# CITlabRostock/citlab-article-separation-new

Measured on AMD Instinct MI355X. Metric: newspaper pages/sec (ARU-Net seg + GNN relation) at 3000x4500 px, higher is better.
Workload: dtype f32s

## Files before the change

### citlab-article-separation-new_amd/csrc/aru_engine.hip

```cpp
#include <algorithm>
#include <cmath>
#include <cstdlib>
#include <memory>

#include "aru_kernels.h"
#include "res8_kernels.h"
#include "res8v_kernels.h"
#include "bf16_kernels.h"
#include "res8w_kernels.h"
#include "convr_kernels.h"
#include "split_kernels.h"
#include "asep_common.h"

using namespace asep;

namespace {

struct Tensor {
    float* p = nullptr;
    int H = 0, W = 0, C = 0;
    bool bf = false;
    size_t count() const { return (size_t)H * W * C; }
    bf16_t* bp() const { return reinterpret_cast<bf16_t*>(p); }
};

struct PackedConv {
    int kh = 0, kw = 0, cin = 0, cout = 0;
    bool c8 = false;
    bool c12 = false;
    bool deconv = false;
    int groups = 0, mtiles = 0, nchunks = 0;
    float* d_w = nullptr;
    float* d_b = nullptr;
    float* d_wino = nullptr;
    float* d_wv = nullptr;
    int bmode = -1;
    int bchunks = 0;
    bf16_t* d_wb = nullptr;
    bf16_t* d_wb8 = nullptr;
    int smode = -1;
    bf16_t* d_ws = nullptr;
    bf16_t* d_ws16 = nullptr;
// ... 15 lines not shown

struct asep_aru {
    asep_aru_cfg cfg{};
    std::map<std::string, PackedConv> convs;
    struct ResB { int C = 0; bf16_t* d_w = nullptr; float* d_b = nullptr; };
    std::map<std::string, ResB> resb;
    bf16_t* d_r8b_down_w = nullptr;
    float* d_r8b_down_b = nullptr;
    bf16_t* d_r8b_up_w1 = nullptr;
    bf16_t* d_r8f_up_w1 = nullptr;
    bf16_t* d_r8f_down_w1 = nullptr;
    float* d_r8b_down_w1r = nullptr;
    bool use_res32 = true;
    int walk_mode = 1;
    bool use_deconvs = true;
    bool use_convr = true;
    unsigned char* d_zero_trash = nullptr;
    int fused_act = 0;
    bool use_walk = true;
    bf16_t* d_r8b_up_w = nullptr;
    float* d_r8b_up_b = nullptr;
    float* d_r8b_up_b1 = nullptr;
    DirectConv det_first, att_first;
    float* d_r8_down_wr = nullptr;
    float* d_r8_down_br = nullptr;
    float* d_r8_up_w1 = nullptr;
    float* d_r8_up_wr = nullptr;
    float* d_r8_up_br = nullptr;
    float* d_r8_up_b1 = nullptr;
    float* d_r8v_down_wr = nullptr;
    float* d_r8v_up_w1 = nullptr;
    float* d_r8v_up_wr = nullptr;
    bool r8_valu = true;
    bool use_fused8 = true;
    bool fused8_wanted = true;
    bool fused8_var = false;
    float* d_att_head = nullptr;
    bf16_t* d_att_headb = nullptr;
    float* d_logit_w = nullptr;
    float* d_logit_b = nullptr;
    float* d_logit_wd = nullptr;
    float* d_stats = nullptr;
    double* d_sums = nullptr;
    struct Lane {
        hipStream_t s = nullptr;
        bool own_stream = false;
        hipStream_t side = nullptr;
        hipEvent_t ev_fork = nullptr, ev_join = nullptr, ev_begin = nullptr, ev_done = nullptr;
        hipStream_t bside = nullptr;
        hipEvent_t ev_bfork = nullptr, ev_bjoin = nullptr;
        BufferPool pool;
        ~Lane() {
            if (ev_fork) (void)hipEventDestroy(ev_fork);
            if (ev_bfork) (void)hipEventDestroy(ev_bfork);
            if (ev_bjoin) (void)hipEventDestroy(ev_bjoin);
            if (ev_join) (void)hipEventDestroy(ev_join);
            if (ev_begin) (void)hipEventDestroy(ev_begin);
            if (ev_done) (void)hipEventDestroy(ev_done);
            if (side) (void)hipStreamDestroy(side);
            if (bside) (void)hipStreamDestroy(bside);
            if (own_stream && s) (void)hipStreamDestroy(s);
        }
    };
    std::vector<std::unique_ptr<Lane>> lanes;
    Lane* cur = nullptr;
    int last_nl = 0;
// ... 732 lines not shown
        if (!rc) rc = upload(pwr, &m->d_r8_up_wr);
        if (!rc) rc = upload(pbr, &m->d_r8_up_br);
        if (!rc) rc = upload(b1->second.data, &m->d_r8_up_b1);
        if (!rc) rc = upload(vw1, &m->d_r8v_up_w1);
        if (!rc) rc = upload(vwr2, &m->d_r8v_up_wr);
        if (rc) return rc;
        m->owned.push_back(m->d_r8v_up_w1); m->owned.push_back(m->d_r8v_up_wr);
        m->owned.push_back(m->d_r8_up_w1); m->owned.push_back(m->d_r8_up_wr);
        m->owned.push_back(m->d_r8_up_br); m->owned.push_back(m->d_r8_up_b1);
        if (hipFuncSetAttribute((const void*)res8_up_kernel<false>, hipFuncAttributeMaxDynamicSharedMemorySize, (int)R8_UP_LDS) != hipSuccess ||
            hipFuncSetAttribute((const void*)res8v_up_kernel<0>, hipFuncAttributeMaxDynamicSharedMemorySize, (int)R8_UP_LDS) != hipSuccess ||
            hipFuncSetAttribute((const void*)res8v_up_kernel<1>, hipFuncAttributeMaxDynamicSharedMemorySize, (int)R8_UP_LDS) != hipSuccess ||
            hipFuncSetAttribute((const void*)res8v_up_kernel<2>, hipFuncAttributeMaxDynamicSharedMemorySize, (int)R8_UP_LDS) != hipSuccess) {
            set_error("cannot reserve %zu bytes of LDS for the fused up block", R8_UP_LDS);
            return ASEP_ERR_HIP;
        }
    }
    if (hipFuncSetAttribute((const void*)res8_down_kernel<false>, hipFuncAttributeMaxDynamicSharedMemorySize, (int)R8_DOWN_LDS) != hipSuccess ||
        hipFuncSetAttribute((const void*)res8v_down_kernel<0>, hipFuncAttributeMaxDynamicSharedMemorySize, (int)R8_DOWN_LDS) != hipSuccess ||
        hipFuncSetAttribute((const void*)res8v_down_kernel<1>, hipFuncAttributeMaxDynamicSharedMemorySize, (int)R8_DOWN_LDS) != hipSuccess ||
        hipFuncSetAttribute((const void*)res8v_down_kernel<2>, hipFuncAttributeMaxDynamicSharedMemorySize, (int)R8_DOWN_LDS) != hipSuccess) {
        set_error("cannot reserve %zu bytes of LDS for the fused residual block", R8_DOWN_LDS);
        return ASEP_ERR_HIP;
    }
    return ASEP_OK;
}

bool r8v_fits(const TL& l) {
    for (const Tensor& t : l)
        if ((size_t)t.H * t.W >= ((size_t)1 << 28)) return false;
    return true;
}

void run_res8_down(asep_aru* m, const TL& imgs, const std::vector<const float*>& stats, bool want_pool, TL* d_out, TL* pool_out) {
    for (const Tensor& t : imgs) {
        d_out->push_back(new_tensor(m, t.H, t.W, 8));
        if (want_pool) pool_out->push_back(new_tensor(m, cdiv(t.H, 2), cdiv(t.W, 2), 8));
    }
    for (size_t b0 = 0; b0 < imgs.size(); b0 += MAXP) {
        const size_t b1 = std::min(imgs.size(), b0 + MAXP);
        Res8Args a{};
        int tiles = 0;
        double flops = 0, bytes = 0;
        for (size_t i = b0; i < b1; ++i) {
            bytes += tbytes(imgs[i]) + tbytes((*d_out)[i]) + (want_pool ? tbytes((*pool_out)[i]) : 0.0);
            Res8Prob& p = a.p[i - b0];
            p.img = imgs[i].p; p.in1 = nullptr; p.stats = stats.empty() ? nullptr : stats[i];
            p.out = (*d_out)[i].p; p.pool = want_pool ? (*pool_out)[i].p : nullptr;
            p.H = imgs[i].H; p.W = imgs[i].W;
            p.tiles_x = cdiv(imgs[i].W, R8_OW);
            p.tile_begin = tiles;
            tiles += p.tiles_x * cdiv(imgs[i].H, R8_OH * R8_NP);
            flops += 2.0 * imgs[i].H * imgs[i].W * (9.0 * 8 + 3 * 9.0 * 64);
        }
        a.nprob = (int)(b1 - b0);
        a.total_tiles = tiles;
        a.w1 = m->det_first.d_w; a.b1 = m->det_first.d_b;
        bool valu = m->r8_valu;
        for (size_t i = b0; i < b1; ++i) valu = valu && (size_t)imgs[i].H * imgs[i].W < ((size_t)1 << 28);
        a.wr = (const f32x4*)(valu ? m->d_r8v_down_wr : m->d_r8_down_wr); a.br = m->d_r8_down_br;
        TL sub(imgs.begin() + b0, imgs.begin() + b1);
        const std::string pname = valu ? std::string("res8v_down_kernel<0>") : std::string("res8_down_kernel<false>");
        ProfScope ps(m, pname, flops, "unet_down_0 (conv1+3xconvR+add+pool) " + dims_of(sub));
        ps.bytes = bytes;
        a.sched = tile_schedule(m, a, std::min(tiles, m->num_cus), R8_OH * R8_NP);
        const dim3 gd(std::min(tiles, m->num_cus));
        const int actv = m->cfg.activation;
        if (actv && !valu) { set_error("level-0 block of an elu / leaky graph: image too large for the vector-ALU kernel"); throw ArgError(); }
        if (valu && actv == 1) { ps.set_name("res8v_down_kernel<1>"); hipLaunchKernelGGL(res8v_down_kernel<1>, gd, dim3(R8_THREADS), R8_DOWN_LDS, m->stream, a); }
        else if (valu && actv == 2) { ps.set_name("res8v_down_kernel<2>"); hipLaunchKernelGGL(res8v_down_kernel<2>, gd, dim3(R8_THREADS), R8_DOWN_LDS, m->stream, a); }
        else if (valu) hipLaunchKernelGGL(res8v_down_kernel<0>, gd, dim3(R8_THREADS), R8_DOWN_LDS, m->stream, a);
        else hipLaunchKernelGGL(res8_down_kernel<false>, gd, dim3(R8_THREADS), R8_DOWN_LDS, m->stream, a);
    }
}

TL run_res8_up(asep_aru* m, const TL& skip, const TL& v) {
    TL out;
    for (const Tensor& t : skip) out.push_back(new_tensor(m, t.H, t.W, 8));
    for (size_t b0 = 0; b0 < skip.size(); b0 += MAXP) {
        const size_t b1 = std::min(skip.size(), b0 + MAXP);
        Res8Args a{};
        int tiles = 0;
        double flops = 0, bytes = 0;
        for (size_t i = b0; i < b1; ++i) {
            bytes += tbytes(skip[i]) + tbytes(v[i]) + tbytes(out[i]);
            Res8Prob& p = a.p[i - b0];
            p.img = skip[i].p; p.in1 = v[i].p; p.stats = nullptr; p.out = out[i].p; p.pool = nullptr;
            p.H = skip[i].H; p.W = skip[i].W;
            p.tiles_x = cdiv(skip[i].W, R8_OW);
            p.tile_begin = tiles;
            tiles += p.tiles_x * cdiv(skip[i].H, R8_OH * R8_NP);
            flops += 2.0 * skip[i].H * skip[i].W * (9.0 * 16 * 8 + 3 * 9.0 * 64);
        }
        a.nprob = (int)(b1 - b0);
        a.total_tiles = tiles;
        bool valu = m->r8_valu;
        for (size_t i = b0; i < b1; ++i) valu = valu && (size_t)skip[i].H * skip[i].W < ((size_t)1 << 28);
        a.w1 = valu ? m->d_r8v_up_w1 : m->d_r8_up_w1; a.b1 = m->d_r8_up_b1;
        a.wr = (const f32x4*)(valu ? m->d_r8v_up_wr : m->d_r8_up_wr); a.br = m->d_r8_up_br;
        TL sub(skip.begin() + b0, skip.begin() + b1);
        const std::string pname = valu ? std::string("res8v_up_kernel<0>") : std::string("res8_up_kernel<false>");
        ProfScope ps(m, pname, flops, "unet_up_0 (conv1[16->8]+3xconvR+add) " + dims_of(sub));
        ps.bytes = bytes;
        a.sched = tile_schedule(m, a, std::min(tiles, m->num_cus), R8_OH * R8_NP);
        const dim3 grid(std::min(tiles, m->num_cus));
        const int actv = m->cfg.activation;
        if (actv && !valu) { set_error("level-0 block of an elu / leaky graph: image too large for the vector-ALU kernel"); throw ArgError(); }
        if (valu && actv == 1) { ps.set_name("res8v_up_kernel<1>"); hipLaunchKernelGGL(res8v_up_kernel<1>, grid, dim3(R8_THREADS), R8_UP_LDS, m->stream, a); }
        else if (valu && actv == 2) { ps.set_name("res8v_up_kernel<2>"); hipLaunchKernelGGL(res8v_up_kernel<2>, grid, dim3(R8_THREADS), R8_UP_LDS, m->stream, a); }
        else if (valu) hipLaunchKernelGGL(res8v_up_kernel<0>, grid, dim3(R8_THREADS), R8_UP_LDS, m->stream, a);
        else hipLaunchKernelGGL(res8_up_kernel<false>, grid, dim3(R8_THREADS), R8_UP_LDS, m->stream, a);
    }
    return out;
}

bf16_t f2bf(float f) {
    uint32_t u;
    memcpy(&u, &f, 4);
    u += 0x7fffu + ((u >> 16) & 1u);
    return (bf16_t)(u >> 16);
}

int upload_bf(const std::vector<bf16_t>& h, bf16_t** d) {
    ASEP_HIP_CHECK(hipMalloc((void**)d, std::max<size_t>(h.size(), 8) * sizeof(bf16_t)));
    ASEP_HIP_CHECK(hipMemcpy(*d, h.data(), h.size() * sizeof(bf16_t), hipMemcpyHostToDevice));
    return ASEP_OK;
}

template <class WF>
void pack_frags_conv(int mode, int kh, int kw, int cin, int mtiles, WF W, std::vector<bf16_t>& dst, int* nchunks) {
    const int taps = kh * kw;
    const int chunks = mode == 0 ? kh : (mode == 1 ? (taps + 1) / 2 : (cin / 32) * taps);
    *nchunks = chunks;
    for (int ch = 0; ch < chunks; ++ch)
        for (int mt = 0; mt < mtiles; ++mt)
            for (int lane = 0; lane < 64; ++lane)
                for (int j = 0; j < 8; ++j) {
// ... 157 lines not shown
        auto bi = blob.find(scope + "/convR_" + std::to_string(r) + "/biases");
        if (wi == blob.end() || bi == blob.end()) { set_error("weights: missing %s/convR_%d", scope.c_str(), r); return ASEP_ERR_WEIGHTS; }
        const HostTensor& w = wi->second;
        if (w.dims.size() != 4 || w.dims[0] != 3 || w.dims[1] != 3 || w.dims[2] != C || w.dims[3] != C) return ASEP_OK;
        auto W = [&](int tap, int ci, int co) -> float { return (ci < C && co < C) ? w.data[((size_t)tap * C + ci) * C + co] : 0.f; };
        int nch = 0;
        if (C == 32) pack_frags_conv(2, 3, 3, 32, 2, W, pk, &nch);
        else pack_frags_conv(C == 8 ? 0 : 1, 3, 3, C, 1, W, pk, &nch);
        br.insert(br.end(), bi->second.data.begin(), bi->second.data.end());
    }
    asep_aru::ResB rb;
    rb.C = C;
    int rc = upload_bf(pk, &rb.d_w);
    if (!rc) rc = upload(br, &rb.d_b);
    if (rc) return rc;
    m->owned.push_back(rb.d_w);
    m->owned.push_back(rb.d_b);
    m->resb[scope] = rb;
    return ASEP_OK;
}

void pack_pair_frags(const HostTensor& w, int cin, std::vector<bf16_t>& dst) {
    const int halves = cin == 16 ? 2 : 1;
    for (int ky = 0; ky < 3; ++ky)
        for (int hf = 0; hf < halves; ++hf)
            for (int lane = 0; lane < 64; ++lane)
                for (int j = 0; j < 8; ++j) {
                    const int m = lane & 15, kk = lane >> 4, e = m >> 3, co = m & 7;
                    const int p = cin == 16 ? 2 * hf + (kk >> 1) : kk;
                    const int ci = cin == 16 ? (kk & 1) * 8 + j : j;
                    const int kx = p - e;
                    dst.push_back(f2bf((kx >= 0 && kx <= 2) ? w.data[(((size_t)ky * 3 + kx) * cin + ci) * 8 + co] : 0.f));
                }
}

int pack_res8b(asep_aru* m, const std::map<std::string, HostTensor>& blob) {
    auto tail = [&](const std::string& scope, bf16_t** d_w, float** d_b) -> int {
        std::vector<bf16_t> pk;
        std::vector<float> br;
        for (int r = 0; r < 3; ++r) {
            auto wi = blob.find(scope + "/convR_" + std::to_string(r) + "/weights");
            auto bi = blob.find(scope + "/convR_" + std::to_string(r) + "/biases");
            if (wi == blob.end() || bi == blob.end()) { set_error("weights: missing %s/convR_%d", scope.c_str(), r); return ASEP_ERR_WEIGHTS; }
            const HostTensor& w = wi->second;
            if (w.dims.size() != 4 || w.dims[0] != 3 || w.dims[1] != 3 || w.dims[2] != 8 || w.dims[3] != 8) return 1;
            pack_pair_frags(w, 8, pk);
            br.insert(br.end(), bi->second.data.begin(), bi->second.data.end());
        }
        int rc = upload_bf(pk, d_w);
        if (!rc) rc = upload(br, d_b);
        if (rc) return rc;
        m->owned.push_back(*d_w);
        m->owned.push_back(*d_b);
        return ASEP_OK;
    };
    int rc = tail("aru_net/featMapG/unet_down_0", &m->d_r8b_down_w, &m->d_r8b_down_b);
    if (rc == 1) { m->d_r8b_down_w = nullptr; return ASEP_OK; }
    if (rc) return rc;
    {
        auto w1 = blob.find("aru_net/featMapG/unet_down_0/conv1/weights");
        if (w1 != blob.end() && w1->second.dims.size() == 4 && w1->second.dims[0] == 3 && w1->second.dims[1] == 3 && w1->second.dims[2] == 1 &&
            w1->second.dims[3] == 8) {
            std::vector<bf16_t> pk;
            for (int lane = 0; lane < 64; ++lane)
                for (int jj = 0; jj < 8; ++jj) {
                    const int mrow = lane & 15, kk = lane >> 4, e = mrow >> 3, co = mrow & 7;
// ... 996 lines not shown
asep_aru* asep_aru_load(const void* weight_blob, size_t nbytes, const asep_aru_cfg* cfg) {
    ASEP_GUARD_BEGIN
    if (!cfg || !weight_blob) { set_error("asep_aru_load: null argument"); return nullptr; }
    if (cfg->struct_size != (int32_t)sizeof(asep_aru_cfg)) {
        set_error("asep_aru_load: cfg.struct_size is %d, this library's asep_aru_cfg has %zu bytes (ABI version %d): the binding was "
                  "written against another include/asep_hip.h", cfg->struct_size, sizeof(asep_aru_cfg), ASEP_ABI_VERSION);
        return nullptr;
    }
    if (cfg->channels != 1) { set_error("asep_aru_load: only 1-channel input is supported (ARU_v1.py:115)"); return nullptr; }
    if (cfg->compute_dtype < 0 || cfg->compute_dtype > 2) { set_error("asep_aru_load: compute_dtype %d unknown (0 = fp32, 1 = bf16 MFMA, 2 = fp32 with split bf16 products)", cfg->compute_dtype); return nullptr; }
    if (cfg->scale_space_num < 1 || cfg->res_depth < 1) { set_error("asep_aru_load: bad cfg"); return nullptr; }
    if (cfg->activation < 0 || cfg->activation > 2) { set_error("asep_aru_load: activation %d unknown (0 = relu, 1 = elu, 2 = leaky)", cfg->activation); return nullptr; }
    const bool variant = cfg->activation != 0 || cfg->plain_u != 0;
    if (cfg->plain_u && cfg->use_attention) { set_error("asep_aru_load: graph 'U' has no attention branch (ARU_v1.py:92-97)"); return nullptr; }
    std::map<std::string, HostTensor> blob;
    if (!parse_blob(weight_blob, nbytes, blob)) return nullptr;
    warn_ignored_switches();
    std::unique_ptr<asep_aru> m(new asep_aru());
    m->cfg = *cfg;
    m->bf16 = cfg->compute_dtype == 1;
    m->split = cfg->compute_dtype == 2;
    if (const char* e = getenv("ASEP_FUSE_POOL")) m->fuse_pool = atoi(e) != 0;
    if (const char* e = getenv("ASEP_FUSE_ACT")) m->fuse_act = atoi(e) != 0;
    if (const char* e = getenv("ASEP_C12")) m->use_c12 = atoi(e) != 0;
    if (const char* e = getenv("ASEP_FUSED8")) m->use_fused8 = atoi(e) != 0;
    m->fused8_wanted = m->use_fused8;
    if (variant) m->use_fused8 = false;
    if (const char* e = getenv("ASEP_R8_VALU")) m->r8_valu = atoi(e) != 0;
    m->fused8_var = variant && !cfg->plain_u && cfg->activation != 0 && m->fused8_wanted && m->r8_valu && m->fuse_act && !m->bf16;
    if (const char* e = getenv("ASEP_XCD_SCHED")) m->use_xcd_sched = atoi(e) != 0;
    if (const char* e = getenv("ASEP_BF_RES32")) m->use_res32 = atoi(e) != 0;
    if (const char* e = getenv("ASEP_BF_CONVR")) m->use_convr = atoi(e) != 0;
    if (const char* e = getenv("ASEP_SPLIT_DECONV")) m->use_deconvs = atoi(e) != 0;
    if (const char* e = getenv("ASEP_BF_WALK")) { m->walk_mode = atoi(e); m->use_walk = m->walk_mode != 0; }
    if (const char* e = getenv("ASEP_LANES")) { m->num_lanes = std::max(1, std::min(4, atoi(e))); m->lanes_forced = true; }
    for (int l = 0; l < m->num_lanes; ++l) {
        std::unique_ptr<asep_aru::Lane> L(new asep_aru::Lane());
        bool ok = hipStreamCreateWithFlags(&L->side, hipStreamNonBlocking) == hipSuccess &&
                  hipStreamCreateWithFlags(&L->bside, hipStreamNonBlocking) == hipSuccess &&
                  hipEventCreateWithFlags(&L->ev_fork, hipEventDisableTiming) == hipSuccess &&
                  hipEventCreateWithFlags(&L->ev_bfork, hipEventDisableTiming) == hipSuccess &&
                  hipEventCreateWithFlags(&L->ev_bjoin, hipEventDisableTiming) == hipSuccess &&
                  hipEventCreateWithFlags(&L->ev_join, hipEventDisableTiming) == hipSuccess &&
                  hipEventCreateWithFlags(&L->ev_begin, hipEventDisableTiming) == hipSuccess &&
                  hipEventCreateWithFlags(&L->ev_done, hipEventDisableTiming) == hipSuccess;
        if (ok && l > 0) { ok = hipStreamCreateWithFlags(&L->s, hipStreamNonBlocking) == hipSuccess; L->own_stream = ok; }
        if (!ok) { set_error("asep_aru_load: cannot create streams/events for lane %d", l); return nullptr; }
        m->lanes.push_back(std::move(L));
    }
    m->cur = m->lanes[0].get();
    int rc = ASEP_OK;
    const int n = cfg->scale_space_num;
    if (cfg->use_attention) {
        rc = pack_direct(m.get(), blob, "aru_net/attMapG/attPart/conv1", &m->att_first);
        if (!rc && m->att_first.k == 4 && m->att_first.cout == 12) {
            const HostTensor& w = blob.find("aru_net/attMapG/attPart/conv1/weights")->second;
            std::vector<float> pk(64 * 4, 0.f);
            for (int lane = 0; lane < 64; ++lane)
                for (int r = 0; r < 4; ++r) {
                    const int co = lane & 15, ky = lane >> 4, kx = r;
                    if (co < 12) pk[lane * 4 + r] = w.data[(size_t)(ky * 4 + kx) * 12 + co];
                }
            rc = upload(pk, &m->d_att_head);
            if (!rc) m->owned.push_back(m->d_att_head);
            if (!rc && m->bf16) {
                std::vector<bf16_t> pb(64 * 8, 0);
                for (int lane = 0; lane < 64; ++lane) {
                    const int co = lane & 15, kk = lane >> 4;
                    for (int i = 0; i < 8 && kk < 2 && co < 12; ++i) pb[lane * 8 + i] = f2bf(w.data[(size_t)((2 * kk + (i >> 2)) * 4 + (i & 3)) * 12 + co]);
                }
                rc = upload_bf(pb, &m->d_att_headb);
                if (!rc) m->owned.push_back(m->d_att_headb);
            }
        }
        for (int i = 2; i <= 4 && !rc; ++i)
            rc = pack_conv(m.get(), blob, "aru_net/attMapG/attPart/conv" + std::to_string(i), "biases", false);
    }
    if (!rc) rc = pack_direct(m.get(), blob, "aru_net/featMapG/unet_down_0/conv1", &m->det_first);
    for (int l = 0; l < n && !rc; ++l) {
        const std::string s = "aru_net/featMapG/unet_down_" + std::to_string(l);
        if (l > 0) rc = pack_conv(m.get(), blob, s + "/conv1", "biases", false);
        if (cfg->plain_u) { if (!rc) rc = pack_conv(m.get(), blob, s + "/conv2", "biases", false); continue; }
        for (int r = 0; r < cfg->res_depth && !rc; ++r)
            rc = pack_conv(m.get(), blob, s + "/convR_" + std::to_string(r), "biases", false);
    }
    for (int l = n - 2; l >= 0 && !rc; --l) {
        const std::string s = "aru_net/featMapG/unet_up_" + std::to_string(l);
        rc = pack_conv(m.get(), blob, s + "/deconv", "bias", true);
        if (!rc) rc = pack_conv(m.get(), blob, s + "/conv1", "biases", false);
        if (cfg->plain_u) { if (!rc) rc = pack_conv(m.get(), blob, s + "/conv2", "biases", false); continue; }
        for (int r = 0; r < cfg->res_depth && !rc; ++r)
            rc = pack_conv(m.get(), blob, s + "/convR_" + std::to_string(r), "biases", false);
    }
    if (!rc && (!variant || m->fused8_var) && !m->bf16 && cfg->feat_root == 8 && cfg->res_depth == 3 && m->det_first.k == 3) rc = pack_res8(m.get(), blob);
    m->fused_act = (m->bf16 && variant && !cfg->plain_u && cfg->activation != 0 && m->fused8_wanted && m->fuse_act) ? cfg->activation : 0;
    const bool fusedb = m->bf16 && (!variant || m->fused_act);
    if (!rc && fusedb && cfg->res_depth == 3 && cfg->feat_root == 8) rc = pack_res8b(m.get(), blob);
    if (!rc && fusedb && cfg->res_depth == 3)
        for (int l = 0; l < n && !rc; ++l) {
            const int f = cfg->feat_root << l;
            if (f != 8 && f != 16 && !(f == 32 && m->use_res32)) continue;
            rc = pack_resb(m.get(), blob, "aru_net/featMapG/unet_down_" + std::to_string(l), f);
            if (!rc && l < n - 1) rc = pack_resb(m.get(), blob, "aru_net/featMapG/unet_up_" + std::to_string(l), f);
        }
    if (rc) return nullptr;
    {
        hipDeviceProp_t prop;
        int dev = 0;
        if (hipGetDevice(&dev) == hipSuccess && hipGetDeviceProperties(&prop, dev) == hipSuccess && prop.multiProcessorCount > 0)
            m->num_cus = prop.multiProcessorCount;
    }
    auto lw = blob.find("aru_net/logit/class/weights");
    auto lb = blob.find("aru_net/logit/class/biases");
    if (lw == blob.end() || lb == blob.end()) { set_error("weights: missing aru_net/logit/class"); return nullptr; }
    const auto& d = lw->second.dims;
    if (d.size() != 4 || d[0] != 4 || d[1] != 4 || d[2] != cfg->feat_root || d[3] != cfg->n_classes) {
        set_error("weights: aru_net/logit/class/weights must be [4,4,%d,%d]", cfg->feat_root, cfg->n_classes);
        return nullptr;
    }
    if (upload(lw->second.data, &m->d_logit_w) || upload(lb->second.data, &m->d_logit_b)) return nullptr;
    m->owned.push_back(m->d_logit_w);
    m->owned.push_back(m->d_logit_b);
    if (cfg->n_classes == 2) {
        const std::vector<float>& w = lw->second.data;
        std::vector<float> wd((size_t)16 * cfg->feat_root + 1);
        for (size_t i = 0; i < (size_t)16 * cfg->feat_root; ++i) wd[i] = w[2 * i + 1] - w[2 * i];
        wd.back() = lb->second.data[1] - lb->second.data[0];
// ... 227 lines not shown
```

### citlab-article-separation-new_amd/csrc/asep_common.hip

```cpp
#include "asep_common.h"
#include <cstdlib>

namespace asep {

static thread_local char g_err[1024] = "";

void set_error(const char* fmt, ...) {
    va_list ap;
    va_start(ap, fmt);
    vsnprintf(g_err, sizeof(g_err), fmt, ap);
    va_end(ap);
}
const char* get_error() { return g_err; }

void warn_ignored_switches() {
    static bool done = false;
    if (done) return;
    done = true;
    static const char* const gone[] = {
        "ASEP_F32_SPLIT", "ASEP_SPLIT_L0", "ASEP_SPLIT_ALDS", "ASEP_SPLIT_TH16", "ASEP_WINOGRAD", "ASEP_WINO_REG", "ASEP_WINO16", "ASEP_BIGTILE",
        "ASEP_BIGTILE2", "ASEP_XCD_ONESHOT", "ASEP_SIDE_STREAM", "ASEP_FUSED8_VAR", "ASEP_BF_TH8", "ASEP_BF_MTB", "ASEP_BF_W8", "ASEP_BF_R8B",
        "ASEP_BF_R8F", "ASEP_CONVS_DBG", "ASEP_R8S_DBG", "ASEP_MAXP24",
#ifndef ASEP_ABLATION
        "ASEP_GNN_BATCH", "ASEP_GNN_LANES",
// ... 55 lines not shown
        }
        ++next_;
        return b.p;
    }
    Buf b{nullptr, 0};
    ASEP_HIP_CHECK_THROW(hipMalloc(&b.p, bytes));
    b.n = bytes;
    bufs_.push_back(b);
    ++next_;
    return b.p;
}

void BufferPool::release() {
    for (auto& b : bufs_)
        if (b.p) (void)hipFree(b.p);
    bufs_.clear();
    next_ = 0;
}

size_t BufferPool::total_bytes() const {
    size_t t = 0;
    for (auto& b : bufs_) t += b.n;
    return t;
}

}

extern "C" {

const char* asep_last_error(void) { return asep::get_error(); }
const char* asep_version(void) { return "asep_hip 0.5 (gfx950)"; }

const char* asep_engine_switches(void) {
    return "ASEP_FUSE_POOL\nASEP_FUSE_ACT\nASEP_C12\nASEP_FUSED8\nASEP_R8_VALU\nASEP_XCD_SCHED\nASEP_BF_RES32\nASEP_BF_WALK\nASEP_BF_CONVR\nASEP_SPLIT_DECONV\nASEP_LANES\nASEP_GNN_STEP\nASEP_GNN_FACTOR"
#ifdef ASEP_ABLATION
           "\nASEP_GNN_BATCH\nASEP_GNN_LANES"
#endif
        ;
}
int asep_abi_version(void) { return ASEP_ABI_VERSION; }

int asep_device_count(void) {
    int n = 0;
    if (hipGetDeviceCount(&n) != hipSuccess) return 0;
    return n;
}

int asep_init(int device_id) {
    int n = 0;
    ASEP_HIP_CHECK(hipGetDeviceCount(&n));
    if (device_id < 0 || device_id >= n) {
        asep::set_error("asep_init: device %d out of range (%d devices)", device_id, n);
        return ASEP_ERR_ARG;
    }
    ASEP_HIP_CHECK(hipSetDevice(device_id));
    hipDeviceProp_t prop;
    ASEP_HIP_CHECK(hipGetDeviceProperties(&prop, device_id));
    if (strncmp(prop.gcnArchName, "gfx950", 6) != 0) {
        asep::set_error("asep_init: device %d is %s; this library is built for gfx950 only", device_id,
                        prop.gcnArchName);
        return ASEP_ERR_UNSUPPORTED;
    }
    return ASEP_OK;
}

void* asep_host_alloc(size_t nbytes) {
    void* p = nullptr;
// ... 25 lines not shown
```

Baseline: 140.3.

## Add split-bf16 MFMA strip-walk kernel for level-0 residual blocks

Adds a new kernel for the level-0 down and up residual blocks in split mode. It walks vertical strips in row bands, keeps intermediate rows in LDS ring buffers, and runs the 3x3 convs on bf16 MFMA using three-way bf16 splits of weights and activations to keep close to fp32 accuracy. The image border is still handled by the existing vector-ALU kernel through a cached list of frame tiles, so each block becomes two launches. This trades VALU FMA work for MFMA throughput, at the cost of extra split arithmetic, an extra launch, and more complex scheduling.

Result: faster. 149.0, median of 6 (+6.2%).

```diff
diff --git a/citlab-article-separation-new_amd/csrc/aru_engine.hip b/citlab-article-separation-new_amd/csrc/aru_engine.hip
--- a/citlab-article-separation-new_amd/csrc/aru_engine.hip
+++ b/citlab-article-separation-new_amd/csrc/aru_engine.hip
@@ -8,6 +8,7 @@
 #include "res8v_kernels.h"
 #include "bf16_kernels.h"
 #include "res8w_kernels.h"
+#include "res8ws_kernels.h"
 #include "convr_kernels.h"
 #include "split_kernels.h"
 #include "asep_common.h"
@@ -89,6 +90,10 @@
     float* d_r8v_up_w1 = nullptr;
     float* d_r8v_up_wr = nullptr;
     bool r8_valu = true;
+    bool use_split_walk = true;
+    bf16_t* d_r8ws_down_w = nullptr;
+    bf16_t* d_r8ws_up_w = nullptr;
+    bf16_t* d_r8ws_up_w1 = nullptr;
     bool use_fused8 = true;
     bool fused8_wanted = true;
     bool fused8_var = false;
@@ -887,6 +892,78 @@
     return true;
 }
 
+bool r8ws_fits(const Tensor& t) {
+    return (t.W - 4 - R8W_X0) / R8W_TW >= 4 && t.H - 4 - R8W_Y0 >= 32 && (size_t)t.H * t.W < ((size_t)1 << 28);
+}
+bool r8ws_on(asep_aru* m) { return m->split && m->use_split_walk && m->r8_valu && m->cfg.activation == 0 && m->d_r8ws_down_w; }
+const int32_t* r8ws_frame_units(asep_aru* m, const Res8Args& a, const std::vector<bool>& walk, int* count) {
+    std::string key = "f";
+    for (int i = 0; i < a.nprob; ++i) key += ":" + std::to_string(a.p[i].H) + "x" + std::to_string(a.p[i].W) + (walk[i] ? "w" : "t");
+    std::vector<int32_t> units;
+    constexpr int UH = R8_OH * R8_NP;
+    for (int i = 0; i < a.nprob; ++i) {
+        const Res8Prob& p = a.p[i];
+        const int ty = cdiv(p.H, UH), tx = p.tiles_x;
+        const int xr = R8W_X0 + R8W_TW * ((p.W - 4 - R8W_X0) / R8W_TW), ye = R8W_Y0 + 2 * ((p.H - 4 - R8W_Y0) / 2);
+        for (int y = 0; y < ty; ++y)
+            for (int x = 0; x < tx; ++x) {
+                const int ux0 = x * R8_OW, ux1 = std::min(ux0 + R8_OW, p.W), uy0 = y * UH, uy1 = std::min(uy0 + UH, p.H);
+                const bool frame = !walk[i] || ux0 < R8W_X0 || ux1 > xr || uy0 < R8W_Y0 || uy1 > ye;
+                if (frame) units.push_back(p.tile_begin + y * tx + x);
+            }
+    }
+    *count = (int)units.size();
+    auto it = m->sched_cache.find(key);
+    if (it != m->sched_cache.end()) return it->second;
+    int32_t* d = nullptr;
+    if (units.empty() || hipMalloc((void**)&d, units.size() * sizeof(int32_t)) != hipSuccess) return nullptr;
+    if (hipMemcpy(d, units.data(), units.size() * sizeof(int32_t), hipMemcpyHostToDevice) != hipSuccess) { (void)hipFree(d); return nullptr; }
+    m->owned.push_back(d);
+    m->sched_cache[key] = d;
+    return d;
+}
+
+void run_res8ws(asep_aru* m, bool up, const Res8Args& a, const std::vector<bool>& walk, const std::string& what) {
+    Res8WSArgs wa{};
+    int n = 0, items = 0;
+    double flops = 0, bytes = 0;
+    long strip_rows = 0;
+    for (int i = 0; i < a.nprob; ++i) {
+        if (!walk[i]) continue;
+        const Res8Prob& q = a.p[i];
+        Res8WSProb& p = wa.p[n++];
+        if (up) { p.skip = q.img; p.dec = q.in1; }
+        else { p.img = q.img; p.stats = q.stats; p.pool = q.pool; }
+        p.out = q.out;
+        p.H = q.H; p.W = q.W;
+        p.n_strips = (p.W - 4 - R8W_X0) / R8W_TW;
+        p.y_end = R8W_Y0 + 2 * ((p.H - 4 - R8W_Y0) / 2);
+        strip_rows += (long)p.n_strips * (p.y_end - R8W_Y0);
+        const double px = (double)p.n_strips * R8W_TW * (p.y_end - R8W_Y0);
+        flops += 2.0 * px * (9.0 * (up ? 16 : 1) * 8 + 3 * 9.0 * 64);
+        bytes += px * ((up ? 64.0 : 4.0) + 32.0 + (p.pool ? 8.0 : 0.0));
+    }
+    if (!n) return;
+    const long slots = 4L * m->num_cus;
+    int band = (int)std::min<long>(256, std::max<long>(32, strip_rows / (6 * slots)));
+    band = (band + 1) & ~1;
+    for (int i = 0; i < n; ++i) {
+        Res8WSProb& p = wa.p[i];
+        p.band = band;
+        p.tile_begin = items;
+        items += p.n_strips * cdiv(p.y_end - R8W_Y0, band);
+    }
+    wa.nprob = n;
+    if (up) { wa.b1 = m->d_r8_up_b1; wa.w1s = (const u32x4*)m->d_r8ws_up_w1; wa.ws = (const u32x4*)m->d_r8ws_up_w; wa.bias = m->d_r8_up_br; }
+    else { wa.b1 = m->det_first.d_b; wa.w1f = m->det_first.d_w; wa.ws = (const u32x4*)m->d_r8ws_down_w; wa.bias = m->d_r8_down_br; }
+    int units = items;
+    wa.xm = oneshot_map(m, items, &units);
+    ProfScope ps(m, up ? "res8ws_kernel<true>" : "res8ws_kernel<false>", flops, what);
+    ps.bytes = bytes;
+    if (up) hipLaunchKernelGGL(res8ws_kernel<true>, dim3(units), dim3(64), 0, m->stream, wa);
+    else hipLaunchKernelGGL(res8ws_kernel<false>, dim3(units), dim3(64), 0, m->stream, wa);
+}
+
 void run_res8_down(asep_aru* m, const TL& imgs, const std::vector<const float*>& stats, bool want_pool, TL* d_out, TL* pool_out) {
     for (const Tensor& t : imgs) {
         d_out->push_back(new_tensor(m, t.H, t.W, 8));
@@ -916,9 +993,29 @@
         a.wr = (const f32x4*)(valu ? m->d_r8v_down_wr : m->d_r8_down_wr); a.br = m->d_r8_down_br;
         TL sub(imgs.begin() + b0, imgs.begin() + b1);
         const std::string pname = valu ? std::string("res8v_down_kernel<0>") : std::string("res8_down_kernel<false>");
+        a.sched = tile_schedule(m, a, std::min(tiles, m->num_cus), R8_OH * R8_NP);
+        if (valu && r8ws_on(m)) {
+            std::vector<bool> walk(a.nprob);
+            bool any = false;
+            for (int i = 0; i < a.nprob; ++i) { walk[i] = r8ws_fits(imgs[b0 + i]); any = any || walk[i]; }
+            if (any) {
+                int nu = 0;
+                Res8Args f = a;
+                f.sched = r8ws_frame_units(m, a, walk, &nu);
+                if (!f.sched) { set_error("level-0 frame schedule: device allocation failed"); throw ArgError(); }
+                f.total_tiles = nu;
+                {
+                    const double share = (double)nu / tiles;
+                    ProfScope ps(m, pname, flops * share, "unet_down_0 frame " + dims_of(sub));
+                    ps.bytes = bytes * share;
+                    hipLaunchKernelGGL(res8v_down_kernel<0>, dim3(std::min(nu, m->num_cus)), dim3(R8_THREADS), R8_DOWN_LDS, m->stream, f);
+                }
+                run_res8ws(m, false, a, walk, "unet_down_0 (conv1+3xconvR+add+pool) " + dims_of(sub));
+                continue;
+            }
+        }
         ProfScope ps(m, pname, flops, "unet_down_0 (conv1+3xconvR+add+pool) " + dims_of(sub));
         ps.bytes = bytes;
-        a.sched = tile_schedule(m, a, std::min(tiles, m->num_cus), R8_OH * R8_NP);
         const dim3 gd(std::min(tiles, m->num_cus));
         const int actv = m->cfg.activation;
         if (actv && !valu) { set_error("level-0 block of an elu / leaky graph: image too large for the vector-ALU kernel"); throw ArgError(); }
@@ -955,9 +1052,29 @@
         a.wr = (const f32x4*)(valu ? m->d_r8v_up_wr : m->d_r8_up_wr); a.br = m->d_r8_up_br;
         TL sub(skip.begin() + b0, skip.begin() + b1);
         const std::string pname = valu ? std::string("res8v_up_kernel<0>") : std::string("res8_up_kernel<false>");
+        a.sched = tile_schedule(m, a, std::min(tiles, m->num_cus), R8_OH * R8_NP);
+        if (valu && r8ws_on(m) && m->d_r8ws_up_w1) {
+            std::vector<bool> walk(a.nprob);
+            bool any = false;
+            for (int i = 0; i < a.nprob; ++i) { walk[i] = r8ws_fits(skip[b0 + i]); any = any || walk[i]; }
+            if (any) {
+                int nu = 0;
+                Res8Args f = a;
+                f.sched = r8ws_frame_units(m, a, walk, &nu);
+                if (!f.sched) { set_error("level-0 frame schedule: device allocation failed"); throw ArgError(); }
+                f.total_tiles = nu;
+                {
+                    const double share = (double)nu / tiles;
+                    ProfScope ps(m, pname, flops * share, "unet_up_0 frame " + dims_of(sub));
+                    ps.bytes = bytes * share;
+                    hipLaunchKernelGGL(res8v_up_kernel<0>, dim3(std::min(nu, m->num_cus)), dim3(R8_THREADS), R8_UP_LDS, m->stream, f);
+                }
+                run_res8ws(m, true, a, walk, "unet_up_0 (conv1[16->8]+3xconvR+add) " + dims_of(sub));
+                continue;
+            }
+        }
         ProfScope ps(m, pname, flops, "unet_up_0 (conv1[16->8]+3xconvR+add) " + dims_of(sub));
         ps.bytes = bytes;
-        a.sched = tile_schedule(m, a, std::min(tiles, m->num_cus), R8_OH * R8_NP);
         const dim3 grid(std::min(tiles, m->num_cus));
         const int actv = m->cfg.activation;
         if (actv && !valu) { set_error("level-0 block of an elu / leaky graph: image too large for the vector-ALU kernel"); throw ArgError(); }
@@ -1181,6 +1298,55 @@
                     const int kx = p - e;
                     dst.push_back(f2bf((kx >= 0 && kx <= 2) ? w.data[(((size_t)ky * 3 + kx) * cin + ci) * 8 + co] : 0.f));
                 }
+}
+
+void pack_pair_split(const HostTensor& w, int cin, int ci0, int ky, std::vector<bf16_t>& dst) {
+    auto bfval = [](bf16_t b) { uint32_t u = (uint32_t)b << 16; float f; memcpy(&f, &u, 4); return f; };
+    std::vector<bf16_t> part[3];
+    for (int lane = 0; lane < 64; ++lane)
+        for (int i = 0; i < 8; ++i) {
+            const int mr = lane & 15, kk = lane >> 4, e = mr >> 3, co = mr & 7, kx = kk - e;
+            const float v = (kx >= 0 && kx <= 2) ? w.data[(((size_t)ky * 3 + kx) * cin + ci0 + i) * 8 + co] : 0.f;
+            const bf16_t h = f2bf(v);
+            const float r = v - bfval(h);
+            const bf16_t mm = f2bf(r);
+            part[0].push_back(h); part[1].push_back(mm); part[2].push_back(f2bf(r - bfval(mm)));
+        }
+    for (int p = 0; p < 3; ++p) dst.insert(dst.end(), part[p].begin(), part[p].end());
+}
+
+int pack_res8ws(asep_aru* m, const std::map<std::string, HostTensor>& blob) {
+    auto tail = [&](const std::string& scope, std::vector<bf16_t>& pk) -> bool {
+        for (int r = 0; r < 3; ++r) {
+            auto wi = blob.find(scope + "/convR_" + std::to_string(r) + "/weights");
+            if (wi == blob.end()) return false;
+            const HostTensor& w = wi->second;
+            if (w.dims.size() != 4 || w.dims[0] != 3 || w.dims[1] != 3 || w.dims[2] != 8 || w.dims[3] != 8) return false;
+            for (int ky = 0; ky < 3; ++ky) pack_pair_split(w, 8, 0, ky, pk);
+        }
+        return true;
+    };
+    std::vector<bf16_t> dw, uw, u1;
+    if (!tail("aru_net/featMapG/unet_down_0", dw)) return ASEP_OK;
+    if (m->cfg.scale_space_num > 1) {
+        const std::string u = "aru_net/featMapG/unet_up_0";
+        auto w1 = blob.find(u + "/conv1/weights");
+        if (!tail(u, uw) || w1 == blob.end()) return ASEP_OK;
+        const HostTensor& w = w1->second;
+        if (w.dims.size() != 4 || w.dims[0] != 3 || w.dims[1] != 3 || w.dims[2] != 16 || w.dims[3] != 8) return ASEP_OK;
+        for (int ky = 0; ky < 3; ++ky)
+            for (int src = 0; src < 2; ++src) pack_pair_split(w, 16, 8 * src, ky, u1);
+        int rc = upload_bf(uw, &m->d_r8ws_up_w);
+        if (rc) return rc;
+        m->owned.push_back(m->d_r8ws_up_w);
+        rc = upload_bf(u1, &m->d_r8ws_up_w1);
+        if (rc) return rc;
+        m->owned.push_back(m->d_r8ws_up_w1);
+    }
+    int rc = upload_bf(dw, &m->d_r8ws_down_w);
+    if (rc) return rc;
+    m->owned.push_back(m->d_r8ws_down_w);
+    return ASEP_OK;
 }
 
 int pack_res8b(asep_aru* m, const std::map<std::string, HostTensor>& blob) {
@@ -2243,6 +2409,7 @@
     if (const char* e = getenv("ASEP_BF_RES32")) m->use_res32 = atoi(e) != 0;
     if (const char* e = getenv("ASEP_BF_CONVR")) m->use_convr = atoi(e) != 0;
     if (const char* e = getenv("ASEP_SPLIT_DECONV")) m->use_deconvs = atoi(e) != 0;
+    if (const char* e = getenv("ASEP_SPLIT_WALK")) m->use_split_walk = atoi(e) != 0;
     if (const char* e = getenv("ASEP_BF_WALK")) { m->walk_mode = atoi(e); m->use_walk = m->walk_mode != 0; }
     if (const char* e = getenv("ASEP_LANES")) { m->num_lanes = std::max(1, std::min(4, atoi(e))); m->lanes_forced = true; }
     for (int l = 0; l < m->num_lanes; ++l) {
@@ -2304,6 +2471,7 @@
             rc = pack_conv(m.get(), blob, s + "/convR_" + std::to_string(r), "biases", false);
     }
     if (!rc && (!variant || m->fused8_var) && !m->bf16 && cfg->feat_root == 8 && cfg->res_depth == 3 && m->det_first.k == 3) rc = pack_res8(m.get(), blob);
+    if (!rc && m->split && !variant && m->d_r8_down_wr) rc = pack_res8ws(m.get(), blob);
     m->fused_act = (m->bf16 && variant && !cfg->plain_u && cfg->activation != 0 && m->fused8_wanted && m->fuse_act) ? cfg->activation : 0;
     const bool fusedb = m->bf16 && (!variant || m->fused_act);
     if (!rc && fusedb && cfg->res_depth == 3 && cfg->feat_root == 8) rc = pack_res8b(m.get(), blob);
diff --git a/citlab-article-separation-new_amd/csrc/asep_common.hip b/citlab-article-separation-new_amd/csrc/asep_common.hip
--- a/citlab-article-separation-new_amd/csrc/asep_common.hip
+++ b/citlab-article-separation-new_amd/csrc/asep_common.hip
@@ -111,7 +111,7 @@
 const char* asep_version(void) { return "asep_hip 0.5 (gfx950)"; }
 
 const char* asep_engine_switches(void) {
-    return "ASEP_FUSE_POOL\nASEP_FUSE_ACT\nASEP_C12\nASEP_FUSED8\nASEP_R8_VALU\nASEP_XCD_SCHED\nASEP_BF_RES32\nASEP_BF_WALK\nASEP_BF_CONVR\nASEP_SPLIT_DECONV\nASEP_LANES\nASEP_GNN_STEP\nASEP_GNN_FACTOR"
+    return "ASEP_FUSE_POOL\nASEP_FUSE_ACT\nASEP_C12\nASEP_FUSED8\nASEP_R8_VALU\nASEP_XCD_SCHED\nASEP_BF_RES32\nASEP_BF_WALK\nASEP_BF_CONVR\nASEP_SPLIT_DECONV\nASEP_SPLIT_WALK\nASEP_LANES\nASEP_GNN_STEP\nASEP_GNN_FACTOR"
 #ifdef ASEP_ABLATION
            "\nASEP_GNN_BATCH\nASEP_GNN_LANES"
 #endif
diff --git a/citlab-article-separation-new_amd/csrc/res8ws_kernels.h b/citlab-article-separation-new_amd/csrc/res8ws_kernels.h
--- /dev/null
+++ b/citlab-article-separation-new_amd/csrc/res8ws_kernels.h
@@ -0,0 +1,310 @@
+#pragma once
+#include "res8w_kernels.h"
+#include "split_kernels.h"
+
+namespace asep {
+
+struct Res8WSProb {
+    const float* skip;
+    const float* dec;
+    const float* img;
+    const float* stats;
+    float* out;
+    float* pool;
+    int H, W;
+    int n_strips;
+    int band;
+    int y_end;
+    int tile_begin;
+};
+struct Res8WSArgs {
+    Res8WSProb p[MAXP];
+    int nprob;
+    const float* b1;
+    const u32x4* w1s;
+    const float* w1f;
+    const u32x4* ws;
+    const float* bias;
+    XcdMap xm;
+};
+
+__device__ __forceinline__ void r8ws_mm6(const u32x4 (&w)[3], const u32x4 (&xa)[3], const u32x4 (&xb)[3], f32x4& ca, f32x4& cb) {
+    ca = mfma_bf16_k32(w[2], xa[0], ca); cb = mfma_bf16_k32(w[2], xb[0], cb);
+    ca = mfma_bf16_k32(w[0], xa[2], ca); cb = mfma_bf16_k32(w[0], xb[2], cb);
+    ca = mfma_bf16_k32(w[1], xa[1], ca); cb = mfma_bf16_k32(w[1], xb[1], cb);
+    ca = mfma_bf16_k32(w[1], xa[0], ca); cb = mfma_bf16_k32(w[1], xb[0], cb);
+    ca = mfma_bf16_k32(w[0], xa[1], ca); cb = mfma_bf16_k32(w[0], xb[1], cb);
+    ca = mfma_bf16_k32(w[0], xa[0], ca); cb = mfma_bf16_k32(w[0], xb[0], cb);
+}
+__device__ __forceinline__ void r8ws_split4(f32x4 v, u32x2& h, u32x2& m, u32x2& l) {
+    unsigned h0, m0, l0, h1, m1, l1;
+    split3_pair(v.x, v.y, h0, m0, l0);
+    split3_pair(v.z, v.w, h1, m1, l1);
+    h = u32x2{h0, h1}; m = u32x2{m0, m1}; l = u32x2{l0, l1};
+}
+
+template <bool UP>
+__global__ __launch_bounds__(64, 1) void res8ws_kernel(const Res8WSArgs a) {
+    constexpr int TW = R8W_TW;
+    constexpr int W0 = TW + 6, W1 = TW + 4, W2 = TW + 2;
+    constexpr int NR = 4, NT = 16;
+    constexpr int PL0 = W0 * 16, PL1 = W1 * 16, PL2 = W2 * 16;
+    constexpr int IMB = UP ? 0 : 4 * 32 * 4;
+    constexpr int R0_OFF = IMB, R1_OFF = R0_OFF + NR * 3 * PL0, R2_OFF = R1_OFF + NR * 3 * PL1, TC_OFF = R2_OFF + NR * 3 * PL2,
+                  TRASH = TC_OFF + NT * TW * 32, LDSB = TRASH + 16;
+    static_assert(LDSB <= 30 * 1024, "four waves per CU with room to spare");
+    __shared__ __attribute__((aligned(16))) unsigned char lds[LDSB];
+
+    const int lane = threadIdx.x;
+    const int j = lane & 15, kk = lane >> 4, e = kk >> 1, ch = (kk & 1) * 4;
+    const int isB = kk & 1;
+    const int c = 2 * j + e;
+    const int item = sched_tile(a.xm);
+    if (item < 0) return;
+    const int pi = prob_of_tile(a, item);
+    const Res8WSProb& P = a.p[pi];
+    const int li = item - P.tile_begin;
+    const int bi = li / P.n_strips, si = li - bi * P.n_strips;
+    const int x0 = R8W_X0 + TW * si;
+    const int Ya = R8W_Y0 + bi * P.band;
+    const int nb = min(P.band, P.y_end - Ya);
+    const int W = P.W;
+
+    constexpr int NF1 = UP ? 18 : 0, NFW = 27;
+    u32x4 wf[NFW], w1[UP ? NF1 : 1];
+    {
+        const u32x4* wl = a.ws + lane;
+#pragma unroll
+        for (int i = 0; i < NFW; ++i) asm volatile("global_load_dwordx4 %0, %1, off" : "=a"(wf[i]) : "v"(wl + i * 64) : "memory");
+        if constexpr (UP) {
+            const u32x4* w1l = a.w1s + lane;
+#pragma unroll
+            for (int i = 0; i < NF1; ++i) asm volatile("global_load_dwordx4 %0, %1, off" : "=a"(w1[i]) : "v"(w1l + i * 64) : "memory");
+        }
+        asm volatile("s_waitcnt vmcnt(0)" ::: "memory");
+#pragma unroll
+        for (int i = 0; i < NFW; ++i) asm volatile("" : "+a"(wf[i]));
+        if constexpr (UP) {
+#pragma unroll
+            for (int i = 0; i < NF1; ++i) asm volatile("" : "+a"(w1[i]));
+        }
+    }
+    auto wpart = [&](int s, int ky, u32x4 (&o)[3]) {
+#pragma unroll
+        for (int p = 0; p < 3; ++p) o[p] = wf[(s * 3 + ky) * 3 + p];
+    };
+    const f32x4 bias1 = *reinterpret_cast<const f32x4*>(a.b1 + ch);
+    f32x4 biasw[3];
+#pragma unroll
+    for (int t = 0; t < 3; ++t) biasw[t] = *reinterpret_cast<const f32x4*>(a.bias + 8 * t + ch);
+
+    const int gxw = min(x0 - 4 + 2 * j + kk, W - 1);
+    const float* __restrict__ skp = P.skip;
+    const float* __restrict__ dcp = P.dec;
+    auto in_row = [&](const float* __restrict__ src, int gy, f32x4& lo, f32x4& hi) {
+        const float* q = src + ((size_t)gy * (size_t)W + (size_t)gxw) * 8;
+        lo = *reinterpret_cast<const f32x4*>(q);
+        hi = *reinterpret_cast<const f32x4*>(q + 4);
+    };
+    float mean = 0.f, inv = 1.f;
+    if constexpr (!UP) {
+        if (P.stats) { mean = P.stats[0]; inv = P.stats[1]; }
+    }
+    const float* __restrict__ imp = P.img;
+    const size_t ioff0 = (size_t)(Ya - 4 + (lane >> 5)) * (size_t)W + (size_t)(x0 - 4 + (lane & 31));
+    auto iload = [&](int p) { return imp[ioff0 + (size_t)p * 2 * (size_t)W]; };
+    float* const iring = reinterpret_cast<float*>(lds);
+    auto istore = [&](float v, int p) { iring[(p & 1) * 64 + lane] = (v - mean) * inv; };
+    float w1v[UP ? 1 : 36];
+    if constexpr (!UP) {
+#pragma unroll
+        for (int t = 0; t < 9; ++t)
+#pragma unroll
+            for (int o = 0; o < 4; ++o) w1v[t * 4 + o] = a.w1f[t * 8 + ch + o];
+    }
+
+    const int p_last = nb / 2 + 3;
+    u32x4 cin[2][2][3] = {};
+    f32x4 nxt[2][2][2];
+    float inx = 0.f;
+    if constexpr (UP) {
+#pragma unroll
+        for (int r = 0; r < 2; ++r) {
+            f32x4 lo, hi;
+            in_row(skp, Ya - 4 + r, lo, hi);
+            split3_x8(lo, hi, cin[r][0][0], cin[r][0][1], cin[r][0][2]);
+            in_row(dcp, Ya - 4 + r, lo, hi);
+            split3_x8(lo, hi, cin[r][1][0], cin[r][1][1], cin[r][1][2]);
+            in_row(skp, Ya - 2 + r, nxt[r][0][0], nxt[r][0][1]);
+            in_row(dcp, Ya - 2 + r, nxt[r][1][0], nxt[r][1][1]);
+        }
+    } else {
+        istore(iload(0), 0);
+        inx = iload(1);
+    }
+
+    const int lcol = r8w_swz(2 * j + kk) * 16;
+    auto whole = [&](u32x2 pa, u32x2 pb) {
+        const auto s0 = __builtin_amdgcn_permlane16_swap(pa.x, pb.x, false, false);
+        const auto s1 = __builtin_amdgcn_permlane16_swap(pa.y, pb.y, false, false);
+        return u32x4{s0[0], s1[0], s0[1], s1[1]};
+    };
+    const int cs = r8w_swz(c) * 16;
+    const bool v0 = j < W0 / 2, v1 = j < W1 / 2, v2 = j < W2 / 2;
+    const bool tvalid = c >= 3 && c < 3 + TW;
+    const int tcol = (tvalid ? c - 3 : 0) * 32 + ch * 4;
+    const int trd = min(c, TW - 1) * 32 + ch * 4;
+    const bool ost = j < TW / 2;
+    float* __restrict__ const outp = P.out;
+    float* __restrict__ const poolp = P.pool;
+    const size_t Wp = (size_t)((W + 1) >> 1);
+
+    auto store_parts = [&](f32x4 ra, f32x4 rb, int roff, int pl, bool valid, int rowa, int rowb) {
+        u32x2 ha, ma, la, hb, mb, lb;
+        r8ws_split4(relu4i(ra), ha, ma, la);
+        r8ws_split4(relu4i(rb), hb, mb, lb);
+        const u32x4 ph = whole(ha, hb), pm = whole(ma, mb), pl_ = whole(la, lb);
+        const int rr = isB ? rowb : rowa;
+        const int base = valid ? roff + rr * 3 * pl + cs : TRASH;
+        const int step = valid ? pl : 0;
+        *reinterpret_cast<u32x4*>(lds + base) = ph;
+        *reinterpret_cast<u32x4*>(lds + base + step) = pm;
+        *reinterpret_cast<u32x4*>(lds + base + 2 * step) = pl_;
+    };
+    auto ring_read = [&](int roff, int pl, int rr, u32x4 (&o)[3]) {
+#pragma unroll
+        for (int p = 0; p < 3; ++p) o[p] = *reinterpret_cast<const u32x4*>(lds + roff + (rr * 3 + p) * pl + lcol);
+    };
+
+    const int K = nb / 2 + 6;
+#pragma unroll 1
+    for (int k = 0; k < K; ++k) {
+        const int i4 = (2 * k) & (NR - 1), i16 = (2 * k) & (NT - 1);
+        const bool do_c1 = k < nb / 2 + 3, do_s1 = k >= 2 && k < nb / 2 + 4, do_s2 = k >= 4 && k < nb / 2 + 5, do_s3 = k >= 6;
+
+        if (do_s3) {
+            u32x4 q[4][3];
+#pragma unroll
+            for (int r = 0; r < 4; ++r) ring_read(R2_OFF, PL2, (i4 + r - 9) & (NR - 1), q[r]);
+            const f32x4 t0 = *reinterpret_cast<const f32x4*>(lds + TC_OFF + ((i16 - 8) & (NT - 1)) * TW * 32 + trd);
+            const f32x4 t1 = *reinterpret_cast<const f32x4*>(lds + TC_OFF + ((i16 - 7) & (NT - 1)) * TW * 32 + trd);
+            f32x4 va = biasw[2], vb = biasw[2];
+#pragma unroll
+            for (int ky = 0; ky < 3; ++ky) {
+                u32x4 w[3];
+                wpart(2, ky, w);
+                r8ws_mm6(w, q[ky], q[ky + 1], va, vb);
+            }
+            va = relu4i(va + t0);
+            vb = relu4i(vb + t1);
+            const int oy = Ya - 12 + 2 * k;
+            if (ost) {
+                float* o = outp + ((size_t)oy * (size_t)W + (size_t)(x0 + c)) * 8 + ch;
+                *reinterpret_cast<f32x4*>(o) = va;
+                *reinterpret_cast<f32x4*>(o + (size_t)W * 8) = vb;
+            }
+            if constexpr (!UP) {
+                if (poolp) {
+                    const f32x4 mv = f32x4{fmaxf(va.x, vb.x), fmaxf(va.y, vb.y), fmaxf(va.z, vb.z), fmaxf(va.w, vb.w)};
+                    float pm[4];
+#pragma unroll
+                    for (int i = 0; i < 4; ++i) {
+                        const unsigned u = __float_as_uint(mv[i]);
+                        const auto s = __builtin_amdgcn_permlane32_swap(u, u, false, false);
+                        pm[i] = fmaxf(__uint_as_float(s[0]), __uint_as_float(s[1]));
+                    }
+                    if (ost && e == 0) {
+                        float* po = poolp + ((size_t)(oy >> 1) * Wp + (size_t)((x0 >> 1) + j)) * 8 + ch;
+                        *reinterpret_cast<f32x4*>(po) = f32x4{pm[0], pm[1], pm[2], pm[3]};
+                    }
+                }
+            }
+        }
+        if (do_s2) {
+            u32x4 q[4][3];
+#pragma unroll
+            for (int r = 0; r < 4; ++r) ring_read(R1_OFF, PL1, (i4 + r - 6) & (NR - 1), q[r]);
+            f32x4 ra = biasw[1], rb = biasw[1];
+#pragma unroll
+            for (int ky = 0; ky < 3; ++ky) {
+                u32x4 w[3];
+                wpart(1, ky, w);
+                r8ws_mm6(w, q[ky], q[ky + 1], ra, rb);
+            }
+            store_parts(ra, rb, R2_OFF, PL2, v2, (i4 - 5) & (NR - 1), (i4 - 4) & (NR - 1));
+        }
+        if (do_s1) {
+            u32x4 q[4][3];
+#pragma unroll
+            for (int r = 0; r < 4; ++r) ring_read(R0_OFF, PL0, (i4 + r - 3) & (NR - 1), q[r]);
+            f32x4 ra = biasw[0], rb = biasw[0];
+#pragma unroll
+            for (int ky = 0; ky < 3; ++ky) {
+                u32x4 w[3];
+                wpart(0, ky, w);
+                r8ws_mm6(w, q[ky], q[ky + 1], ra, rb);
+            }
+            store_parts(ra, rb, R1_OFF, PL1, v1, (i4 - 2) & (NR - 1), (i4 - 1) & (NR - 1));
+        }
+        if (do_c1) {
+            f32x4 ra = bias1, rb = bias1;
+            if constexpr (UP) {
+                u32x4 x2[2][2][3];
+#pragma unroll
+                for (int r = 0; r < 2; ++r)
+#pragma unroll
+                    for (int s = 0; s < 2; ++s) split3_x8(nxt[r][s][0], nxt[r][s][1], x2[r][s][0], x2[r][s][1], x2[r][s][2]);
+                if (k + 2 <= p_last) {
+#pragma unroll
+                    for (int r = 0; r < 2; ++r) {
+                        in_row(skp, Ya + 2 * k + r, nxt[r][0][0], nxt[r][0][1]);
+                        in_row(dcp, Ya + 2 * k + r, nxt[r][1][0], nxt[r][1][1]);
+                    }
+                }
+#pragma unroll
+                for (int ky = 0; ky < 3; ++ky)
+#pragma unroll
+                    for (int s = 0; s < 2; ++s) {
+                        u32x4 w[3];
+#pragma unroll
+                        for (int p = 0; p < 3; ++p) w[p] = w1[(ky * 2 + s) * 3 + p];
+                        u32x4 xa[3], xb[3];
+#pragma unroll
+                        for (int p = 0; p < 3; ++p) {
+                            xa[p] = ky == 0 ? cin[0][s][p] : (ky == 1 ? cin[1][s][p] : x2[0][s][p]);
+                            xb[p] = ky == 0 ? cin[1][s][p] : (ky == 1 ? x2[0][s][p] : x2[1][s][p]);
+                        }
+                        r8ws_mm6(w, xa, xb, ra, rb);
+                    }
+#pragma unroll
+                for (int r = 0; r < 2; ++r)
+#pragma unroll
+                    for (int s = 0; s < 2; ++s)
+#pragma unroll
+                        for (int p = 0; p < 3; ++p) cin[r][s][p] = x2[r][s][p];
+            } else {
+                istore(inx, k + 1);
+                if (k + 2 <= p_last) inx = iload(k + 2);
+                const int cb = min(c, 29);
+#pragma unroll
+                for (int ky = 0; ky < 3; ++ky)
+#pragma unroll
+                    for (int kx = 0; kx < 3; ++kx) {
+                        const float va = iring[((2 * k + ky) & 3) * 32 + cb + kx], vb = iring[((2 * k + 1 + ky) & 3) * 32 + cb + kx];
+#pragma unroll
+                        for (int o = 0; o < 4; ++o) {
+                            ra[o] = fmaf(va, w1v[(ky * 3 + kx) * 4 + o], ra[o]);
+                            rb[o] = fmaf(vb, w1v[(ky * 3 + kx) * 4 + o], rb[o]);
+                        }
+                    }
+            }
+            if (tvalid) {
+                *reinterpret_cast<f32x4*>(lds + TC_OFF + ((i16 + 1) & (NT - 1)) * TW * 32 + tcol) = ra;
+                *reinterpret_cast<f32x4*>(lds + TC_OFF + ((i16 + 2) & (NT - 1)) * TW * 32 + tcol) = rb;
+            }
+            store_parts(ra, rb, R0_OFF, PL0, v0, (i4 + 1) & (NR - 1), (i4 + 2) & (NR - 1));
+        }
+    }
+}
+
+}
```
